# szemenyeim/DynEnv

Measured on AMD Instinct MI355X. Metric: agent-steps/s, higher is better.
Workload: dtype f64

## Files before the change

dynenv_amd/csrc/driving_kernels.hip:

```cpp
#include "driving_dev.h"

__constant__ DrvConst C;

#include "driving_host.h"

struct DrvMailbox {
  double p1x[DRV_NS][2], p1y[DRV_NS][2], p2x[DRV_NS][2], p2y[DRV_NS][2], nx[DRV_NS], ny[DRV_NS];
  int hash[DRV_NS][2], count[DRV_NS], flag[DRV_NS];
};
struct DrvObsStage {
  float carRow[DRV_MAXA][8];
  float goal[DRV_MAXA][2];
  float shared[DRV_MAXO * 4 + DRV_MAXP * 2 + DRV_LANE_ROWS * 5];
};
#ifdef DRV_PROFILE
#define DRV_PROF(...) __VA_ARGS__
#else
#define DRV_PROF(...)
#endif
#define DRV_CLIST 128
struct __align__(16) DrvLds {
  double px[DRV_NB], py[DRV_NB], vx[DRV_NB], vy[DRV_NB], ang[DRV_NB], w[DRV_NB], vbx[DRV_NB], vby[DRV_NB], wb[DRV_NB];
  double minv[DRV_NB], iinv[DRV_NB];
  double rc[DRV_MAXA], rs[DRV_MAXA], rotAng[DRV_MAXA];
  double dirx[DRV_MAXA], diry[DRV_MAXA], prevx[DRV_MAXA], prevy[DRV_MAXA], goalx[DRV_MAXA], goaly[DRV_MAXA];
  double cosRel0[DRV_MAXA];
  double dprev[DRV_MAXA];
  double cmass[DRV_MAXA], cpower[DRV_MAXA], chx[DRV_MAXA], chy[DRV_MAXA];
  double aabb[DRV_MAXA][4];
  V2 cv[DRV_MAXA][4];
  int flags[DRV_NB], moving[DRV_NB];
  double ox[DRV_MAXO], oy[DRV_MAXO];
  int s_pair[DRV_NS], s_meta[DRV_NS], s_hash0[DRV_NS], s_hash1[DRV_NS];
  double s_jn0[DRV_NS], s_jt0[DRV_NS], s_jn1[DRV_NS], s_jt1[DRV_NS];
  double rewAcc[DRV_MAXA], posAcc[DRV_MAXA];
  int lastCand[64];
  int stepErr;
  unsigned char act[16];
  int still[DRV_NB];
  unsigned short clist[DRV_CLIST];
  int clistN;
  int sLvMeta;
  unsigned long long sActive;
  unsigned char sLevel[DRV_NS];
  union {
    DrvMailbox mb;
    DrvObsStage ob;
  } u;
};

static_assert(sizeof(DrvLds) <= 10240, "16 one-wave workgroups per CU - one residency round of 4096 environments on 256 CUs - need <= 160 KB / 16 of LDS each");
__shared__ DrvLds g_L;


#define DRV_COS_PI_2 6.123233995736766e-17
template <int R>
struct RoadK;
template <>
struct RoadK<0> {
  static constexpr double p0x = 875.0, p0y = 0.0, dirx = 0.0, diry = 1.0, lat = 2.0 * 35.0 + 5.0, length = 1000.0;
  static constexpr double dirAngle = 1.5707963267948966, cosDir0 = DRV_COS_PI_2, nx = -1.0, ny = DRV_COS_PI_2;
};
template <>
struct RoadK<1> {
  static constexpr double p0x = 0.0, p0y = 500.0, dirx = 1.0, diry = 0.0, lat = 1.0 * 35.0 + 5.0, length = 1750.0;
  static constexpr double dirAngle = 0.0, cosDir0 = 1.0, nx = DRV_COS_PI_2, ny = 1.0;
};

struct CarK {
  static constexpr double carMass0 = 1200.0, carMass1 = 1800.0, carMass2 = 3500.0, carMass3 = 5000.0;
  static constexpr double carHx0 = 10.0, carHx1 = 15.0, carHx2 = 20.0, carHx3 = 25.0;
  static constexpr double carHy0 = 5.0, carHy1 = 6.0, carHy2 = 7.0, carHy3 = 8.0;
  static constexpr double carPower0 = 3.0, carPower1 = 4.0, carPower2 = 3.0, carPower3 = 4.0;
  static constexpr double carInertia0 = 50000.0, carInertia1 = 156600.0, carInertia2 = 0x1.ff8e555555555p+18, carInertia3 = 0x1.185ad55555555p+20;
  static constexpr double pedMass = 90.0, pedInertia = 90.0 * (0.5 * (0.0 * 0.0 + DRV_PED_R * DRV_PED_R) + 0.0);
};

template <int R>
DE_DEV int road_pos(V2 point, double cosRel) {
  V2 pt = vsub(point, v2(RoadK<R>::p0x, RoadK<R>::p0y));
  double dist = vcross(v2(RoadK<R>::dirx, RoadK<R>::diry), pt);
// ... 746 lines not shown
      if (active && myLevel == lv && a_state != ARB_FIRST) {
        BodyV a, b;
        body_load(L, bodyA, a);
        body_load(L, bodyB, b);
        arb_warm_start(a, b, n, r1, r2, jn, jt, a_count);
        body_store_vel(L, bodyA, a);
        body_store_vel(L, bodyB, b);
      }
      __syncthreads();
    }
    BodyV a, b;
    bool biasOnly = true;
    if (active) {
      body_load(L, bodyA, a); body_load(L, bodyB, b);
      biasOnly = arb_is_bias_only(a, b, jn, jt, bounce, a_count);
    }
    const int nSteps = maxLevel + 1 + period * 9;
    int due = myLevel, passes = 0;
DRV_PROF(profMode = wave_ballot(!biasOnly) == 0ull ? 3 : 4;)
    if (wave_ballot(!biasOnly) == 0ull) {
      const int ra = body_rd(bodyA), rb = body_rd(bodyB), wa = body_wr(bodyA), wb_ = body_wr(bodyB);
      for (int t = 0; t < nSteps; ++t) {
        if (active && t == due && passes < 10) {
          a.vb = v2(L.vbx[ra], L.vby[ra]); a.wb = L.wb[ra];
          b.vb = v2(L.vbx[rb], L.vby[rb]); b.wb = L.wb[rb];
          arb_apply_bias_only(a, b, n, r1, r2, nMass, bias, jBias, a_count);
          L.vbx[wa] = a.vb.x; L.vby[wa] = a.vb.y; L.wb[wa] = a.wb;
          L.vbx[wb_] = b.vb.x; L.vby[wb_] = b.vb.y; L.wb[wb_] = b.wb;
          due += period; ++passes;
        }
        __syncthreads();
      }
    } else [[unlikely]] {
DRV_PROF(if (lane == 0 && blockIdx.x < 4096) { unsigned long long* d = g_dbgp + blockIdx.x * 8; const unsigned long long P3 = __builtin_amdgcn_s_memtime(); d[2] += P1 - P0; d[3] += (P2 - P1) + ((P3 - P2) << 32); })
      const int bits3 = (restIn ? B3_REST_IN : 0) | (bias[0] == 0.0 ? B3_BIAS0_ZERO : 0) | (bias[1] == 0.0 ? B3_BIAS1_ZERO : 0);
      DrvSolveRet r;
      r[0] = nMass[0]; r[1] = nMass[1]; r[2] = bias[0]; r[3] = bias[1]; r[4] = bounce[0]; r[5] = bounce[1];
      r[6] = jn[0]; r[7] = jn[1]; r[8] = jt[0]; r[9] = jt[1];
      r[10] = drv_pack2(pk, a_pair);
      r[11] = drv_pack2(SOLVE_NEEDS_SPLIT | (bits3 << SR_BITS3_SH) | (myLevel << SR_LEVEL_SH), bodyA | (bodyB << 8) | (maxLevel_ << SR_LVWORD_SH));
      return r;
    }
  }
DRV_PROF(const unsigned long long P3 = __builtin_amdgcn_s_memtime();)
  const int bits = drv_slot_verdicts(lane, pk, a_pair, restIn, bias[0] == 0.0, bias[1] == 0.0, jn[0], jn[1], jt[0], jt[1], jBias[0], jBias[1], false);
DRV_PROF(if (lane == 0 && blockIdx.x < 4096) { unsigned long long* d = g_dbgp + blockIdx.x * 8; const unsigned long long P4 = __builtin_amdgcn_s_memtime(); d[2] += (P1 - P0) + ((P4 - P3) << 32); d[3] += (P2 - P1) + ((P3 - P2) << 32); })
  DrvSolveRet r;
  r[11] = drv_pack2(bits DRV_PROF(| (prof_any(profMode) << SOLVE_PROF_SH)), 0);
  return r;
}
DE_OOL int drv_prestep_solve(int lane, int nCarPed, int pk, int a_pair, int bodyA, int bodyB, int anyActive_, double jn0, double jn1, double jt0,
                             double jt1) {
  return __double2loint(drv_prestep_solve_body<false>(lane, nCarPed, pk, a_pair, bodyA, bodyB, 0, 1 << 8 , anyActive_, jn0, jn1, jt0, jt1)[11]);
}
DE_OOL DrvSolveRet drv_prestep_solve_multi(int lane, int nCarPed, int pk, int a_pair, int bodyA, int bodyB, int myLevel, int maxLevel_, double jn0,
                                           double jn1, double jt0, double jt1) {
  return drv_prestep_solve_body<true>(lane, nCarPed, pk, a_pair, bodyA, bodyB, myLevel, maxLevel_, 1, jn0, jn1, jt0, jt1);
}
DE_OOL int drv_split_verdicts(int lane, int pk, int a_pair, int bits3, double jn0, double jn1, double jBias0, double jBias1, double jt0, double jt1) {
  return drv_slot_verdicts(lane, pk, a_pair, (bits3 & B3_REST_IN) != 0, (bits3 & B3_BIAS0_ZERO) != 0, (bits3 & B3_BIAS1_ZERO) != 0, jn0, jn1, jt0, jt1, jBias0, jBias1, true);
}
enum { CRET_OVERFLOW = 1, CRET_INERT_SH = 1, CRET_INERT = 1 << CRET_INERT_SH, CRET_STEADY_SH = 2, CRET_STEADY = 1 << CRET_STEADY_SH,
       CRET_LIGHT_REPLAY_SH = 3, CRET_LIGHT_REPLAY = 1 << CRET_LIGHT_REPLAY_SH, CRET_SPLIT_SH = 4, CRET_SPLIT = 1 << CRET_SPLIT_SH };
static_assert(SOLVE_ALL_INERT == CRET_INERT && SOLVE_ALL_STEADY == CRET_STEADY && (SOLVE_TOOK_SPLIT << 1) == CRET_SPLIT,
              "drv_contact_path passes the two verdicts on in place and the split bit one place up");
struct ContactRet {
  uint64_t occ;
  int err;
};

DE_DEV ContactRet drv_contact_path(int lane, int cand, int dirty, int light, int A, int nCarPed, uint64_t occ) {
  const bool isCar = lane < A, isPed = lane >= DRV_SLOT_PED && lane < DRV_SLOT_PED + (nCarPed >> 8);
  DrvLds& L = g_L;
  int err = 0;
  asm volatile("" : "+v"(lane));
DRV_PROF(const unsigned long long T0 = __builtin_amdgcn_s_memtime();)
  DrvMailbox& M = L.u.mb;
  if (lane < DRV_NS) M.flag[lane] = 0;
  __syncthreads();
// ... 67 lines not shown
    if (mode == 0) { lightBad = lightBad || touch; continue; }
    const uint64_t tmask = wave_ballot(touch);
    if (tmask == 0ull) continue;
    const bool needNew = touch && slot < 0;
    const uint64_t newMask = wave_ballot(needNew);
    if (newMask) {
      const uint64_t slotBits = (1ull << DRV_NS) - 1ull;
      int rank = __popcll(newMask & ((1ull << lane) - 1ull));
      uint64_t fm = (~occ) & slotBits;
      if (needNew) {
        for (int r = 0; r < rank; ++r) fm &= fm - 1;
        if (fm) { slot = __builtin_ctzll(fm); L.s_pair[slot] = pr; }
        else err |= CRET_OVERFLOW;
      }
      int cnt = __popcll(newMask);
      uint64_t fm2 = (~occ) & slotBits;
      for (int r = 0; r < cnt && fm2; ++r) { occ |= (fm2 & (~fm2 + 1)); fm2 &= fm2 - 1; }
      spair = lane < DRV_NS ? L.s_pair[lane] : -1;
    }
    if (touch && slot >= 0) {
      M.flag[slot] = needNew ? 3 : 1;
      M.count[slot] = ct.count;
      M.nx[slot] = ct.n.x; M.ny[slot] = ct.n.y;
      M.p1x[slot][0] = ct.p1[0].x; M.p1y[slot][0] = ct.p1[0].y; M.p2x[slot][0] = ct.p2[0].x; M.p2y[slot][0] = ct.p2[0].y;
      M.hash[slot][0] = ct.hash[0];
      if (ct.count > 1) {
        M.p1x[slot][1] = ct.p1[1].x; M.p1y[slot][1] = ct.p1[1].y; M.p2x[slot][1] = ct.p2[1].x; M.p2y[slot][1] = ct.p2[1].y;
        M.hash[slot][1] = ct.hash[1];
      }
    }
    __syncthreads();
  }
  __syncthreads();
DRV_PROF(if (lane == 0 && blockIdx.x < 4096) { unsigned long long* d = g_dbgl + blockIdx.x * 8; d[6] += (N1 - T0) + (nMath << 32); d[7] += __builtin_amdgcn_s_memtime() - N1 - nMath; })
  if (mode == 0 && wave_ballot(lightBad) == 0ull) { lightOk = true; break; }
  }
  if (lightOk) {
    ContactRet ret;
    ret.occ = occ; ret.err = err | CRET_LIGHT_REPLAY;
    return ret;
  }

DRV_PROF(const unsigned long long T1 = __builtin_amdgcn_s_memtime();)
  const bool slotOcc = lane < DRV_NS && ((occ >> lane) & 1ull);
  bool touched = false;
  int bodyA = 0, bodyB = 0;
  int a_pair = 0xFFFF, a_state = ARB_FIRST, a_count = 0, a_age = 0;
  bool hashSame = false;
  bool prevSteady = false, prevInert = false;
  double jn[2] = {0.0, 0.0}, jt[2] = {0.0, 0.0};
  V2 n = v2(0.0, 0.0), r1[2], r2[2];
  r1[0] = r1[1] = r2[0] = r2[1] = v2(0.0, 0.0);
  const int sl = lane < DRV_NS ? lane : 0;
  int flag = M.flag[sl], cnt = M.count[sl], h0 = M.hash[sl][0], mh1 = M.hash[sl][1];
  int s_pair = L.s_pair[sl], meta = L.s_meta[sl], oh0 = L.s_hash0[sl], oh1 = L.s_hash1[sl];
  double o_jn0 = L.s_jn0[sl], o_jt0 = L.s_jt0[sl], o_jn1 = L.s_jn1[sl], o_jt1 = L.s_jt1[sl];
  asm volatile("" : "+v"(flag), "+v"(cnt), "+v"(h0), "+v"(mh1), "+v"(s_pair), "+v"(meta), "+v"(oh0), "+v"(oh1), "+v"(o_jn0), "+v"(o_jt0), "+v"(o_jn1), "+v"(o_jt1));
  if (slotOcc) {
    touched = flag != 0;
    a_pair = s_pair;
    a_state = SLOT_STATE(meta); a_count = SLOT_COUNT(meta); a_age = SLOT_AGE(meta);
    prevSteady = SLOT_BIT(meta, META_STEADY_SH); prevInert = SLOT_BIT(meta, META_INERT_SH);
    if (flag & 2) { a_state = ARB_FIRST; a_count = 0; a_age = 0; prevSteady = false; prevInert = false; }
    if (touched) {
      const int i = a_pair >> 8, j = a_pair & 0xFF;
      if (j >= DRV_SLOT_PED && j < DRV_SLOT_OBST) { bodyA = j; bodyB = i; } else { bodyA = i; bodyB = j; }
      const V2 pa = bodyA < DRV_SLOT_OBST ? v2(L.px[bodyA], L.py[bodyA]) : static_pos(L, bodyA);
// ... 104 lines not shown
  else if (nActive > 1 && lvHit) {
    myLevel = c_level;
    maxLevel = (int)(signed char)(uniform_i(c_meta) & 0xFF);
    period = uniform_i(c_meta) >> 8;
  } else if (nActive > 1) {
    if (!haveRank && nTouched > 1)
      for (uint64_t mm = touchedMask; mm; mm &= mm - 1) {
        int b = __builtin_ctzll(mm);
        int pk = bcast_i(a_pair, b);
        rank += (pk < a_pair) ? 1 : 0;
      }
    int bl = 0;
    const int bodyAB = bodyA | (bodyB << 8);
    for (int k = 0; k < nTouched; ++k) {
      uint64_t who = wave_ballot(active && rank == k);
      if (who == 0ull) continue;
      int b = __builtin_ctzll(who);
      const int ab = bcast_i(bodyAB, b), ba = ab & 0xFF, bb2 = ab >> 8;
      const int pa = ba < DRV_SLOT_OBST ? bcast_i(bl, ba) : 0, pb = bb2 < DRV_SLOT_OBST ? bcast_i(bl, bb2) : 0;
      const int la = pa & 0xFF, lb = pb & 0xFF;
      int lv = la > lb ? la : lb;
      const int fa = (pa >> 8) - 1, fb = (pb >> 8) - 1;
      const int lo = fa < 0 ? fb : (fb < 0 ? fa : (fa < fb ? fa : fb));
      if (lo >= 0 && lv - lo + 1 > period) period = lv - lo + 1;
      if (lane == b) myLevel = lv;
      if (lane == ba || lane == bb2) bl = (lv + 1) | (((bl >> 8) ? (bl >> 8) : lv + 1) << 8);
      maxLevel = lv > maxLevel ? lv : maxLevel;
    }
    if (lane < DRV_NS) L.sLevel[lane] = (unsigned char)myLevel;
    if (lane == 0) L.sLvMeta = (maxLevel & 0xFF) | (period << 8);
  }

DRV_PROF(const unsigned long long T2 = __builtin_amdgcn_s_memtime();)
DRV_PROF(if (lane == 0 && blockIdx.x < 4096) { unsigned long long* d = g_dbgs + blockIdx.x * 8; d[0] += U1 - T1; d[1] += U2 - U1; d[2] += U3 - U2; d[3] += U4 - U3; d[4] += T2 - U4; })
  const int pkArg = pk_pack(a_state, a_count, a_age, touched, freeMe, hashSame, prevInert, skipped, slotOcc, active);
  int solveBits;
  if (activeMask == 0ull || maxLevel == 0) {
    solveBits = drv_prestep_solve(lane, nCarPed, pkArg, a_pair, bodyA, bodyB, activeMask != 0ull ? 1 : 0, jn[0], jn[1], jt[0], jt[1]);
  } else {
    const DrvSolveRet sv = drv_prestep_solve_multi(lane, nCarPed, pkArg, a_pair, bodyA, bodyB, myLevel, (maxLevel & 0xFF) | (period << 8), jn[0], jn[1], jt[0], jt[1]);
    solveBits = __double2loint(sv[11]);
    if (uniform_i(solveBits) & SOLVE_NEEDS_SPLIT) [[unlikely]] {
      const int w1 = __double2hiint(sv[11]);
DRV_PROF(const unsigned long long S0 = __builtin_amdgcn_s_memtime();)
      const DrvSplitRet sr = drv_solve_general_split(fresh_lane(), (solveBits >> SR_LEVEL_SH) & 0xFF, w1 & 0xFFFF, w1 >> SR_LVWORD_SH, sv[0], sv[1], sv[2], sv[3], sv[4], sv[5],
                                                     sv[6], sv[7], sv[8], sv[9], __double2loint(sv[10]), __double2hiint(sv[10]), (solveBits >> SR_BITS3_SH) & 7);
DRV_PROF(const unsigned long long S1 = __builtin_amdgcn_s_memtime();)
      solveBits = drv_split_verdicts(fresh_lane(), sr.pk, sr.pair, sr.bits, sr.jn0, sr.jn1, sr.jb0, sr.jb1, sr.jt0, sr.jt1) DRV_PROF(| (4 << SOLVE_PROF_SH));
DRV_PROF(if (fresh_lane() == 0 && blockIdx.x < 4096) { unsigned long long* d = g_dbgp + blockIdx.x * 8; d[3] += (S1 - S0) << 32; d[2] += (__builtin_amdgcn_s_memtime() - S1) << 32; })
    }
  }
  occ &= ~freeMask;
DRV_PROF(const unsigned long long T3 = T2, T4 = T2, T5 = __builtin_amdgcn_s_memtime(); const int profModeW = (uniform_i(solveBits) >> SOLVE_PROF_SH) & 7;)
DRV_PROF(if (lane == 0 && blockIdx.x < 4096) {
  unsigned long long* d = g_dbgp + blockIdx.x * 8;
  d[0] += T1 - T0; d[1] += T2 - T1; d[2] += T3 - T2; d[3] += T4 - T3; d[4] += T5 - T4;
  d[5] += 1ull + (light ? (1ull << 16) : 0ull);
  d[6] += (unsigned long long)(maxLevel + 1) + ((unsigned long long)(maxLevel + 1) << (12 * profModeW));
  d[7] += (unsigned long long)nTouched + ((unsigned long long)profCand << 16);
})
  {
    ContactRet ret;
    ret.occ = occ; ret.err = err | (uniform_i(solveBits) & (SOLVE_ALL_INERT | SOLVE_ALL_STEADY)) | ((uniform_i(solveBits) & SOLVE_TOOK_SPLIT) << 1);
    return ret;
  }
}

DE_OOL int drv_partial_obs_fused(PvIn in, uint64_t seed, int A, int* envi, int env_id_offset, int e, int nPedObst, int elapsed,
                                 uint32_t episode, int noiseTypeAgents, double magn, float* __restrict__ obs, int budgetCycles);
#ifndef DRV_DEFER_MIN_CONTACT
#define DRV_DEFER_MIN_CONTACT 5
#endif
#ifndef DRV_PV_DEADLINE_PCT
#define DRV_PV_DEADLINE_PCT 110
#endif
#ifndef DRV_FUSED_AGENTS
#define DRV_FUSED_AGENTS 10
#endif
enum { LR_MOVING = 1, LR_REMOVED = 2, LR_CAND_CHANGED = 4 };
enum { LS_VB_VALID = 1, LS_AABB_VALID = 2 };
struct DrvLightRet {
  int cand, dirty, bits;
};
DE_OOL DrvLightRet drv_light_substep(int it_, int lane, int A_, int nPed_, int nObst_, int elapsed_,
                                                      uint32_t seedLo, uint32_t seedHi, uint32_t genv_, uint32_t episode_, int stateBits) {
  DrvLds& L = g_L;
DRV_PROF(const unsigned long long Q0 = __builtin_amdgcn_s_memtime();)
  const int lastCand = L.lastCand[lane];
  const int it = uniform_i(it_), A = uniform_i(A_), nPed = uniform_i(nPed_), nObst = uniform_i(nObst_), elapsed = uniform_i(elapsed_);
  const uint32_t genv = (uint32_t)uniform_i((int)genv_), episode = (uint32_t)uniform_i((int)episode_);
  const uint64_t seed = ((uint64_t)(uint32_t)uniform_i((int)seedHi) << 32) | (uint64_t)(uint32_t)uniform_i((int)seedLo);
  const bool isCar = lane < A;
  const bool isPed = lane >= DRV_SLOT_PED && lane < DRV_SLOT_PED + nPed;
  const bool isBody = isCar || isPed;
  const bool vbValid = (uniform_i(stateBits) & LS_VB_VALID) != 0;
  bool aabbValid = (uniform_i(stateBits) & LS_AABB_VALID) != 0;
    bool turned = false;
    const int bi = lane & (DRV_NB - 1), ci = lane < DRV_MAXA ? lane : DRV_MAXA - 1;
    int f = L.flags[bi];
    double px = L.px[bi], py = L.py[bi], vx = L.vx[bi], vy = L.vy[bi], ang = L.ang[bi];
    const double w = L.w[bi];
    const double vbx = vbValid ? L.vbx[bi] : 0.0, vby = vbValid ? L.vby[bi] : 0.0, wb = vbValid ? L.wb[bi] : 0.0;
    double rcv = L.rc[ci], rsv = L.rs[ci], rotAngv = L.rotAng[ci], cosRel0v = L.cosRel0[ci];
    const double goalx = L.goalx[ci], goaly = L.goaly[ci], dprev = L.dprev[ci], chx = L.chx[ci], chy = L.chy[ci];
    double rew = L.rewAcc[ci], posrew = L.posAcc[ci];
    int moving = L.moving[bi];
    if (!isBody) { f = 0; px = 0.0; py = 0.0; vx = 0.0; vy = 0.0; }
    if (isCar) {
      if (it == 0) {
        const int actPk = (int)L.act[lane];
        const int acc = (actPk & 3) - 1, steer = ((actPk >> 2) - 1) * 2;
        if (!CARF_FIN(f)) {
          double dirx = L.dirx[lane], diry = L.diry[lane];
          double power = (double)acc;
          double moveDir = vx * dirx + vy * diry;
          bool skip = false;
          if (acc < 0) power = (double)acc * 0.75;
          if (acc == 0) power = (moveDir == 0.0) ? 0.0 : (moveDir > 0.0 ? -2.0 : 2.0);
          else if (acc < 0 && moveDir > 0.0) skip = true;
          else if (acc > 0 && moveDir < 0.0) skip = true;
          if (!skip) {
            const double cs = rcv, sn = rsv;
            const double cpower = L.cpower[lane];
            vx = vx + cpower * power * cs;
            vy = vy + cpower * power * sn;
            if (acc == 0 && (vx * dirx + vy * diry) * moveDir < 0.0) { vx = 0.0; vy = 0.0; }
          }
          if (steer != 0) {
            const double rot = (double)steer * (DM_PI / 180.0);
            ang = ang + rot;
            const DevSC rsc = dev_sincos_inl(rot);
            const double sn = rsc.s, cs = rsc.c;
            const double dx = dirx * cs - diry * sn, dy = dirx * sn + diry * cs;
            L.dirx[lane] = dx; L.diry[lane] = dy;
            const double nvx = vx * cs - vy * sn, nvy = vx * sn + vy * cs;
            vx = nvx; vy = nvy;
            L.ang[lane] = ang;
            const CarRot cr = car_refresh_rot<true>(L, lane, ang);
            rcv = cr.c; rsv = cr.s; rotAngv = ang; cosRel0v = cr.cosRel0;
            turned = true;
// ... 4 lines not shown
DRV_PROF(const unsigned long long Q1 = __builtin_amdgcn_s_memtime();)
    const V2 pos = v2(px, py);
    int lp = LP_OffRoad;
    if (isBody) {
      int rp = road_pos<0>(pos, isCar ? cosRel0v : RoadK<0>::cosDir0);
      if (rp < lp) lp = rp;
      rp = road_pos<1>(pos, isCar ? rcv : RoadK<1>::cosDir0);
      if (rp < lp) lp = rp;
    }
DRV_PROF(const unsigned long long Q2 = __builtin_amdgcn_s_memtime();)
    if (isCar) {
      const double dnow = vlen(vsub(pos, v2(goalx, goaly)));
      const double diff = dprev - dnow;
      if (!CARF_FIN(f)) { const double d50 = diff / 50.0; rew += d50; posrew += dm_max(0.0, d50); }
      L.prevx[lane] = px; L.prevy[lane] = py; L.dprev[lane] = dnow;
      if (lp >= LP_OverRoad) {
        if (!CARF_FIN(f)) {
          if (lp == LP_OverRoad && dnow < 100.0) {
            lp = LP_AtGoal;
            f |= CARF_FIN_BIT | CARF_FRIC_BIT;
            rew += (double)(DRV_MAX_TIME - elapsed) / 100.0;
            posrew += (double)(DRV_MAX_TIME - elapsed) / 100.0;
          } else {
            f |= CARF_CRASH_BITS;
            rew -= vlen(v2(vx, vy)) / 5.0;
          }
        }
      } else if (lp == LP_InOpposingLane) {
        if (!CARF_FIN(f)) rew -= vlen(v2(vx, vy)) / 10000.0;
      }
      f = CARF_SET_LP(f, lp);
      if (px >= DRV_W + 50.0 || px <= -50.0 || py >= DRV_H + 50.0 || py <= -50.0) { vx = 0.0; vy = 0.0; }
      L.flags[lane] = f;
      L.vx[lane] = vx; L.vy[lane] = vy;
      L.rewAcc[lane] = rew; L.posAcc[lane] = posrew;
DRV_PROF(asm volatile("" ::: "memory");)
    } else if (isPed) {
      if (!PEDF_DEAD(f)) {
        int crossing = PEDF_CROSSING(f), beginc = PEDF_BEGIN(f), side = PEDF_SIDE(f);
        const bool isOffRoad = lp >= LP_OverRoad;
        const bool isOut = drv_is_out(pos);
        if (moving > 0) {
          moving = (moving - DRV_TIME_DIFF > 0) ? moving - DRV_TIME_DIFF : 0;
          if (crossing) {
            if (!beginc && isOffRoad) { moving = 0; crossing = 0; vx = 0.0; vy = 0.0; }
            else if (beginc && !isOffRoad) { beginc = 0; }
          }
          if (isOut) { moving = 0; vx = 0.0; vy = 0.0; }
        } else {
          if (!crossing) {
            dm_u32x4 u = dm_env_rng(seed, genv, episode, DM_RNG_PED_MOVE, (uint32_t)(lane - DRV_SLOT_PED), (uint32_t)elapsed);
            const bool r1 = PEDF_ROAD(f) != 0;
            const V2 rdir = r1 ? v2(RoadK<1>::dirx, RoadK<1>::diry) : v2(RoadK<0>::dirx, RoadK<0>::diry);
            const V2 rnrm = r1 ? v2(RoadK<1>::nx, RoadK<1>::ny) : v2(RoadK<0>::nx, RoadK<0>::ny);
            V2 dir = rdir;
            moving = dm_randint(u.v[0], 5000, 30000);
            int speed = dm_randint(u.v[1], -2, 2);
            if (!isOffRoad) {
              crossing = 1; beginc = 0;
              if (speed == 0) speed = 2;
            } else if (isOut) {
              dir = drv_is_out(vadd(pos, rdir)) ? vneg(rdir) : rdir;
            } else if (dm_unit(u.v[2]) < 0.05) {
              crossing = 1; beginc = 1;
              dir = side ? rnrm : vneg(rnrm);
              side = side ? 0 : 1;
              speed = dm_randint(u.v[3], 1, 2);
            }
            const V2 nv = vmul(vmul(dir, (double)PEDF_SPEED(f)), (double)speed);
            vx = nv.x; vy = nv.y;
          } else if (isOffRoad) {
            crossing = 0; beginc = 0;
          }
        }
        L.moving[lane] = moving;
        L.flags[lane] = PEDF_PACK(PEDF_ROAD(f), side, 0, crossing, beginc, PEDF_SPEED(f));
        L.vx[lane] = vx; L.vy[lane] = vy;
      }
    }

DRV_PROF(const unsigned long long Q3 = __builtin_amdgcn_s_memtime();)
    double bl = 0.0, bb = 0.0, br = -1.0, bt = -1.0;
    bool live = false;
    int sj = 3;
    if (isBody) {
      const double npx = px + (vx + vbx) * DE_DT, npy = py + (vy + vby) * DE_DT, nang = ang + (w + wb) * DE_DT;
      const bool still = !turned && vx == 0.0 && vy == 0.0 && w == 0.0 && vbx == 0.0 && vby == 0.0 && wb == 0.0;
      L.px[lane] = npx; L.py[lane] = npy; L.ang[lane] = nang;
      const bool frozen = !turned && vx == 0.0 && vy == 0.0 && w == 0.0 && npx == px && npy == py && nang == ang;
      sj = (still ? 1 : 0) | (frozen ? 2 : 0);
      L.still[lane] = sj;
      live = true;
      if (isCar) {
        if (nang != rotAngv) { const CarRot cr = car_refresh_rot<true>(L, lane, nang); rcv = cr.c; rsv = cr.s; }
        if (!aabbValid || !frozen) {
          BoxW bw;
          box_world(bw, v2(npx, npy), rcv, rsv, chx, chy);
          double l = INFINITY, r = -INFINITY, b = INFINITY, t = -INFINITY;
#pragma unroll
          for (int k = 0; k < 4; ++k) {
            l = fmin_cp(l, bw.v[k].x); r = fmax_cp(r, bw.v[k].x); b = fmin_cp(b, bw.v[k].y); t = fmax_cp(t, bw.v[k].y);
          }
          bl = l - 0.0; bb = b - 0.0; br = r + 0.0; bt = t + 0.0;
#pragma unroll
          for (int k = 0; k < 4; ++k) L.cv[lane][k] = bw.v[k];
          L.aabb[lane][0] = bl; L.aabb[lane][1] = bb; L.aabb[lane][2] = br; L.aabb[lane][3] = bt;
        } else {
          bl = L.aabb[lane][0]; bb = L.aabb[lane][1]; br = L.aabb[lane][2]; bt = L.aabb[lane][3];
        }
      } else {
// ... 1 lines not shown
      }
    } else if (lane >= DRV_SLOT_OBST && lane < DRV_SLOT_BLD + 4) {
      live = lane >= DRV_SLOT_BLD || (lane - DRV_SLOT_OBST) < nObst;
      const V2 c = static_pos(L, lane);
      const double ex = lane >= DRV_SLOT_BLD ? DRV_BLD_HX : DRV_OBST_H, ey = lane >= DRV_SLOT_BLD ? DRV_BLD_HY : DRV_OBST_H;
      bl = -ex + c.x; br = ex + c.x; bb = -ey + c.y; bt = ey + c.y;
    }
    aabbValid = true;
    __syncthreads();
DRV_PROF(const unsigned long long Q4 = __builtin_amdgcn_s_memtime();)

    int cand = 0;
    bool candMoving = false, removed = false;
    int dirty = 0;
    {
      const int carStill = (int)(wave_ballot(isCar && (sj & 1)) & 0x3FFull);
      const int carFrozen = (int)(wave_ballot(isCar && (sj & 2)) & 0x3FFull);
#pragma unroll
      for (int i = 0; i < DRV_MAXA; ++i) {
        const double al = L.aabb[i][0], ab = L.aabb[i][1], ar = L.aabb[i][2], at = L.aabb[i][3];
        const bool hit = (al <= br) & (bl <= ar) & (ab <= bt) & (bb <= at);
        cand |= hit ? (1 << i) : 0;
      }
      {
        const int lim = lane < A ? lane : A;
        cand &= live ? ((1 << lim) - 1) : 0;
      }
      if (cand) candMoving = !(sj & 1) || (cand & ~carStill) != 0;
      const int clean = (lastCand >= 0 && (sj & 2)) ? (cand & lastCand & carFrozen) : 0;
      dirty = cand & ~clean;
      removed = lastCand < 0 || (lastCand & ~cand) != 0;
    }
  L.lastCand[lane] = cand;
DRV_PROF(if (lane == 0 && blockIdx.x < 4096) {
  unsigned long long* d = g_dbgl + blockIdx.x * 8;
  const unsigned long long Q5 = __builtin_amdgcn_s_memtime();
  if (it == 0) { for (int k = 0; k < 8; ++k) d[k] = 0ull; }
  d[0] += Q1 - Q0; d[1] += Q2 - Q1; d[2] += Q3 - Q2; d[3] += Q4 - Q3; d[4] += Q5 - Q4; d[5] += Q5 - Q0;
})
  DrvLightRet ret;
  ret.cand = cand; ret.dirty = dirty; ret.bits = (candMoving ? LR_MOVING : 0) | (removed ? LR_REMOVED : 0) | (cand != lastCand ? LR_CAND_CHANGED : 0);
  return ret;
}
DE_DEV unsigned drv_hw_simd_key() {
  const unsigned hw = (unsigned)__builtin_amdgcn_s_getreg(63492) , xcc = (unsigned)__builtin_amdgcn_s_getreg(63508) ;
  return ((xcc & 0xFu) << 16) | (hw & 0xFF30u);
}
DE_DEV int drv_launch_tick(const DrvState& S) { return S.tick_src ? uniform_i(__atomic_load_n(&S.iso[DRV_ISOW_TICK], __ATOMIC_RELAXED)) : S.tick; }
DE_DEV int drv_launch_pv(const DrvState& S) { return S.tick_src ? uniform_i(__atomic_load_n(&S.iso[DRV_ISOW_PV_PAR], __ATOMIC_RELAXED)) : S.pv_par; }
DE_DEV int drv_iso_assign(const DrvState& S, int lane, int tick) {
  const int b = blockIdx.x, E = S.E;
  if (!S.iso_on) return b;
  const int buf = tick % 3;
  if (b == 0 && lane == 0) { const int nn = (tick + 2) % 3; S.iso[DRV_ISOW_LEN + nn] = 0; S.iso[DRV_ISOW_SLOWEST + nn] = 0; }
  if (S.iso_on == 3) return b;
  int K = uniform_i(S.iso[DRV_ISOW_LEN + buf]);
  const int cap = S.iso_on == 1 ? DRV_ISO_MAX : DRV_ISO_LIST;
  K = K < cap ? K : cap;
  const int G = S.iso_on == 1 ? 4 * DRV_ISO_GROUPS : E;
  if (S.iso_on == 1) {
    if (b < G) { if (lane == 0) S.iso_hw[(size_t)(tick & 1) * (4 * DRV_ISO_GROUPS) + b] = drv_hw_simd_key(); }
    else if (b == G + 3 * DRV_ISO_MAX) {
      const unsigned* hw = S.iso_hw + (size_t)((tick + 1) & 1) * (4 * DRV_ISO_GROUPS);
      bool bad = false;
      for (int g = DRV_ISO_G0 + lane; g < DRV_ISO_G0 + DRV_ISO_GSPAN; g += 64) {
        const unsigned k0 = hw[g], k1 = hw[g + DRV_ISO_GROUPS], k2 = hw[g + 2 * DRV_ISO_GROUPS], k3 = hw[g + 3 * DRV_ISO_GROUPS];
        bad |= k0 == 0xFFFFFFFFu || k0 != k1 || k0 != k2 || k0 != k3;
      }
      const bool ok = wave_ballot(bad) == 0ull;
      if (lane == 0) {
        int cd = S.iso[DRV_ISOW_COOL];
        if (!ok) cd = DRV_ISO_COOLDOWN; else if (cd > 0) cd -= 1;
        S.iso[DRV_ISOW_COOL] = cd;
        S.iso[DRV_ISOW_VALID + (tick + 1) % 3] = (ok && cd == 0) ? 1 : 0;
// ... 47 lines not shown
#endif
#ifndef DRV_ISO_PCT
#define DRV_ISO_PCT 75
#endif
DE_DEV void drv_iso_report(const DrvState& S, int e, int lane, unsigned long long t0, int tick) {
  if (!S.iso_on || lane != 0) return;
  const int cycles = (int)(__builtin_amdgcn_s_memtime() - t0);
  const int buf = tick % 3, nxt = (tick + 1) % 3;
  const int slowest = S.iso[DRV_ISOW_SLOWEST + buf];
  if (cycles > DRV_ISO_MIN && cycles > (slowest / 100) * DRV_ISO_PCT) atomicMax(&S.iso[DRV_ISOW_SLOWEST + nxt], cycles);
  if (S.iso_on == 3) return;
  if (slowest > DRV_ISO_MIN && cycles > (slowest / 100) * DRV_ISO_PCT) {
    const int k = atomicAdd(&S.iso[DRV_ISOW_LEN + nxt], 1);
    if (k < DRV_ISO_LIST) S.iso[DRV_ISO_HDR + nxt * DRV_ISO_LIST + k] = e;
  }
  __atomic_store_n(&S.iso_done[e], tick, __ATOMIC_RELAXED);
}

template <bool PARTIAL>
DE_DEV void drv_step_body(const DrvState& S, const uint8_t* __restrict__ mask, const int* __restrict__ actions, float* __restrict__ obs,
                          double* __restrict__ rewards, uint8_t* __restrict__ dones, float* __restrict__ pobs, int pvNoise, double pvMagn) {
  const unsigned long long isoT0 = __builtin_amdgcn_s_memtime();
DRV_PROF(const unsigned long long KS = isoT0;)
  DrvLds& L = g_L;
  int lane = threadIdx.x;
  const int tick = drv_launch_tick(S);
  if (!S.tick_src && blockIdx.x == 0 && lane == 0) { S.iso[DRV_ISOW_TICK] = S.tick; S.iso[DRV_ISOW_PV_PAR] = S.pv_par; }
  const int e = drv_iso_assign(S, lane, tick);
  if (e < 0) return;
  if (mask && uniform_i(mask[e]) == 0) {
    if ((S.iso_on == 1 || S.iso_on == 2) && lane == 0) __atomic_store_n(&S.iso_done[e], tick, __ATOMIC_RELAXED);
    return;
  }
DRV_PROF(if (lane < 8 && e < 4096) { g_dbgp[e * 8 + lane] = 0ull; g_dbgs[e * 8 + lane] = 0ull; })
  const int A = S.A;
  int* envi = S.envi + (size_t)e * EI_COUNT;
  int elapsed = uniform_i(envi[EI_ELAPSED]);
  int allFinished = uniform_i(envi[EI_ALLFIN]);
  const int nPed = uniform_i(envi[EI_NPED]);
  const int nObst = uniform_i(envi[EI_NOBST]);
  const uint32_t episode = (uint32_t)uniform_i(envi[EI_EPISODE]);
  uint64_t occ = (uint64_t)(uint32_t)uniform_i(envi[EI_OCC]);
  if (occ != 0ull) __builtin_amdgcn_s_setprio(3);
  else if (PARTIAL) __builtin_amdgcn_s_setprio(1);
  const uint32_t genv = (uint32_t)(S.env_id_offset + e);

  const bool isCar = lane < A;
  const bool isPed = lane >= DRV_SLOT_PED && lane < DRV_SLOT_PED + nPed;
  const bool isBody = isCar || isPed;
  const int g_act0 = actions[((size_t)e * A + (isCar ? lane : 0)) * 2 + 0], g_act1 = actions[((size_t)e * A + (isCar ? lane : 0)) * 2 + 1];
  const int g_lastCand = S.lastcand[(size_t)e * 64 + lane];
  load_env(S, L, e, lane, A, nPed, nObst, occ);

  {
    int act0 = isCar ? g_act0 : 1, act1 = isCar ? g_act1 : 1;
    const bool bad = (unsigned)act0 > 2u || (unsigned)act1 > 2u;
    if (bad) { act0 = 1; act1 = 1; }
    if (lane < 16) L.act[lane] = (unsigned char)(act0 | (act1 << 2));
    const bool anyBad = wave_ballot(bad) != 0ull;
    if (lane == 0) L.stepErr = anyBad ? DYNENV_ERRBIT_ACTION : 0;
  }
  int finishedAt = -1;
  if (lane < DRV_MAXA) { L.rewAcc[lane] = 0.0; L.posAcc[lane] = 0.0; }
  bool aabbValid = false;
  L.lastCand[lane] = g_lastCand;
  if (lane == 0) { L.clistN = -1; L.sActive = ~0ull; L.sLvMeta = 0; }
  bool inertAll = (uniform_i(envi[EI_SHORTCUT]) & SC_INERT) != 0;
  bool steadyAll = (uniform_i(envi[EI_SHORTCUT]) & SC_STEADY) != 0;
  bool vbValid = (uniform_i(envi[EI_SHORTCUT]) & SC_VB_VALID) != 0;
  unsigned cntA = 0u, cntB = 0u;
#define DRV_CNT(ei) (1u << (4 * ((ei) - EI_N_FAST)))
#define DRV_CNT_GET(ei) ((int)((cntA >> (4 * ((ei) - EI_N_FAST))) & 15u))
  static_assert(EI_N_STEADY - EI_N_FAST == 7 && EI_N_SLOTS - EI_N_FAST == 3 && DRV_NS * 10 < 256, "seven counters of four bits in cntA, the slot sum in eight bits of cntB");
  __syncthreads();

DRV_PROF(const unsigned long long K0 = __builtin_amdgcn_s_memtime(); unsigned long long tPh1 = 0, tBroad = 0, tFast = 0, tCont = 0, tBook = 0;)
  bool lightOff = false;
  for (int it = 0; it < 10; ++it) {
    lane = fresh_lane();
DRV_PROF(const unsigned long long A0 = __builtin_amdgcn_s_memtime();)
    const DrvLightRet lr = drv_light_substep(it, lane, A, nPed, nObst, elapsed, (uint32_t)S.seed, (uint32_t)(S.seed >> 32), genv, episode,
                                             (vbValid ? LS_VB_VALID : 0) | (aabbValid ? LS_AABB_VALID : 0));
    const int cand = lr.cand, dirty = lr.dirty;
    const bool candMoving = (lr.bits & LR_MOVING) != 0, removed = (lr.bits & LR_REMOVED) != 0;
    aabbValid = true;
DRV_PROF(const unsigned long long A1 = A0;)
    const uint64_t anyCand = wave_ballot(cand != 0);
    const bool candChanged = wave_ballot((lr.bits & LR_CAND_CHANGED) != 0) != 0ull, anyMoving = wave_ballot(candMoving) != 0ull;
    if (candChanged && lane == 0) L.clistN = -1;
    const bool quiescent = inertAll && !candChanged && !anyMoving;
    const bool steadyOk = !quiescent && steadyAll && wave_ballot(removed) == 0ull;
    const bool anyDirty = wave_ballot(dirty != 0) != 0ull;
    bool replay = steadyOk && !anyDirty;
    const bool light = steadyOk && anyDirty && !lightOff;
    if (!(anyCand == 0ull && occ == 0ull) && !quiescent && !replay) cntA += candChanged ? DRV_CNT(EI_N_WHY_CAND) : anyMoving ? DRV_CNT(EI_N_WHY_MOVING) : DRV_CNT(EI_N_WHY_INERT);

DRV_PROF(const unsigned long long A2 = __builtin_amdgcn_s_memtime(); bool tookContact = false;)
    cntA += (anyCand == 0ull && occ == 0ull) ? DRV_CNT(EI_N_FAST) : quiescent ? DRV_CNT(EI_N_QUIET) : replay ? DRV_CNT(EI_N_STEADY) : DRV_CNT(EI_N_CONTACT);
    cntB += (unsigned)__popcll(occ);
    if ((anyCand == 0ull && occ == 0ull) || quiescent) {
      velocity_update_ool(A | (nPed << 8));
      if (anyCand == 0ull && occ == 0ull) steadyAll = false;
      vbValid = false;
    } else if (!replay) {
DRV_PROF(tookContact = true;)
      __builtin_amdgcn_s_setprio(3);
      ContactRet cr = drv_contact_path(lane, cand, dirty, light ? 1 : 0, A, A | (nPed << 8), occ);
      lane = fresh_lane();
      if (wave_ballot((cr.err & CRET_OVERFLOW) != 0) != 0ull && lane == 0) L.stepErr |= DYNENV_ERRBIT_OVERFLOW;
      if (light && !(uniform_i(cr.err >> CRET_LIGHT_REPLAY_SH) & 1)) lightOff = true;
      if (uniform_i(cr.err >> CRET_LIGHT_REPLAY_SH) & 1) {
        replay = true; cntB = (unsigned)uniform_i((int)(cntB + (1u << 8)));
      } else {
        cntB = (unsigned)uniform_i((int)(cntB + ((unsigned)(uniform_i(cr.err >> CRET_SPLIT_SH) & 1) << 12)));
        occ = uniform_u64(cr.occ);
        inertAll = (uniform_i(cr.err >> CRET_INERT_SH) & 1) != 0;
        steadyAll = (uniform_i(cr.err >> CRET_STEADY_SH) & 1) != 0;
        vbValid = true;
      }
    }
    if (replay) {
      velocity_update_ool(A | (nPed << 8));
      vbValid = true;
    }
    __syncthreads();
    if (!PARTIAL) lane = fresh_lane();

DRV_PROF(const unsigned long long A3 = __builtin_amdgcn_s_memtime(); tPh1 += A1 - A0; tBroad += A2 - A1; if (tookContact) tCont += A3 - A2; else tFast += A3 - A2;)
    elapsed += 1;
    bool notDone = false;
    if (isCar) { int f = L.flags[lane]; notDone = !(CARF_FIN(f) && !CARF_CRASHED(f)); }
    const bool allFin = wave_ballot(notDone) == 0ull;
    if (!allFinished && allFin) {
      allFinished = 1;
      finishedAt = elapsed;
    }
  }
  lane = fresh_lane();
  const double teamReward = finishedAt >= 0 ? 0.0 + (double)(DRV_MAX_TIME - finishedAt) / 100.0 : 0.0;

DRV_PROF(const unsigned long long K1 = __builtin_amdgcn_s_memtime();)
  double* er = S.epr + (size_t)e * 16 + (isCar ? lane : 0);
  double* ep = S.epr + (size_t)S.E * 16 + (size_t)e * 16 + (isCar ? lane : 0);
  const double g_er = *er, g_ep = *ep;
  const int cl = lane < 10 ? lane : 0;
  const int g_cnt = envi[EI_N_FAST + cl];
  const int g_err = envi[EI_ERR];
  double rew = 0.0, posrew = 0.0;
  if (isCar) {
    rew = L.rewAcc[lane] + teamReward;
    posrew = L.posAcc[lane] + dm_max(0.0, teamReward);
    rewards[(size_t)e * A + lane] = rew;
  }
  if (lane == 0) {
    dones[e] = (uint8_t)(elapsed >= DRV_MAX_TIME);
    envi[EI_ELAPSED] = elapsed; envi[EI_ALLFIN] = allFinished; envi[EI_OCC] = (int)(uint32_t)occ;
    envi[EI_SHORTCUT] = (inertAll ? SC_INERT : 0) | (steadyAll ? SC_STEADY : 0) | (vbValid ? SC_VB_VALID : 0);
  }
  const int errBits = uniform_i(L.stepErr);
  S.lastcand[(size_t)e * 64 + lane] = L.lastCand[lane];
  store_env(S, L, e, lane, A, nPed, occ);
  if (obs) write_full_obs_ool(lane, A, nPed, nObst, S.obs_dim, obs + (size_t)e * A * S.obs_dim);
  if (isCar) { *er = g_er + rew; *ep = g_ep + posrew; }
  {
    static_assert(EI_N_QUIET == EI_N_FAST + 1 && EI_N_CONTACT == EI_N_FAST + 2 && EI_N_SLOTS == EI_N_FAST + 3 && EI_N_WHY_CAND == EI_N_FAST + 4 &&
                  EI_N_WHY_MOVING == EI_N_FAST + 5 && EI_N_WHY_INERT == EI_N_FAST + 6 && EI_N_STEADY == EI_N_FAST + 7 && EI_N_LIGHT == EI_N_FAST + 8 && EI_N_SPLIT == EI_N_FAST + 9,
// ... 215 lines not shown
```

Before: 272.9 million.

## Fuse velocity update and path decisions into light substep, drop per-step barrier

The velocity/friction update for the fast, quiescent and replay paths now runs inside the light substep, and that function computes the wave-uniform path decision bits. This removes a separate out-of-line velocity_update call, the vx/vy round trip through LDS, and the per-iteration __syncthreads. The all-finished check is deferred to the next substep through a ballot on previous flags, plus one final check after the loop. The profiling index now comes from an LDS env id instead of blockIdx. The risk is subtle ordering changes: w is written before the broadphase reads it, and correctness now depends on a compiler memory barrier rather than an explicit sync.

```diff
diff --git a/dynenv_amd/csrc/driving_kernels.hip b/dynenv_amd/csrc/driving_kernels.hip
--- a/dynenv_amd/csrc/driving_kernels.hip
+++ b/dynenv_amd/csrc/driving_kernels.hip
@@ -47,6 +47,7 @@
     DrvMailbox mb;
     DrvObsStage ob;
   } u;
+DRV_PROF(int profEnv;)
 };
 
 static_assert(sizeof(DrvLds) <= 10240, "16 one-wave workgroups per CU - one residency round of 4096 environments on 256 CUs - need <= 160 KB / 16 of LDS each");
@@ -859,7 +860,7 @@
         __syncthreads();
       }
     } else [[unlikely]] {
-DRV_PROF(if (lane == 0 && blockIdx.x < 4096) { unsigned long long* d = g_dbgp + blockIdx.x * 8; const unsigned long long P3 = __builtin_amdgcn_s_memtime(); d[2] += P1 - P0; d[3] += (P2 - P1) + ((P3 - P2) << 32); })
+DRV_PROF(if (lane == 0 && g_L.profEnv < 4096) { unsigned long long* d = g_dbgp + g_L.profEnv * 8; const unsigned long long P3 = __builtin_amdgcn_s_memtime(); d[2] += P1 - P0; d[3] += (P2 - P1) + ((P3 - P2) << 32); })
       const int bits3 = (restIn ? B3_REST_IN : 0) | (bias[0] == 0.0 ? B3_BIAS0_ZERO : 0) | (bias[1] == 0.0 ? B3_BIAS1_ZERO : 0);
       DrvSolveRet r;
       r[0] = nMass[0]; r[1] = nMass[1]; r[2] = bias[0]; r[3] = bias[1]; r[4] = bounce[0]; r[5] = bounce[1];
@@ -871,7 +872,7 @@
   }
 DRV_PROF(const unsigned long long P3 = __builtin_amdgcn_s_memtime();)
   const int bits = drv_slot_verdicts(lane, pk, a_pair, restIn, bias[0] == 0.0, bias[1] == 0.0, jn[0], jn[1], jt[0], jt[1], jBias[0], jBias[1], false);
-DRV_PROF(if (lane == 0 && blockIdx.x < 4096) { unsigned long long* d = g_dbgp + blockIdx.x * 8; const unsigned long long P4 = __builtin_amdgcn_s_memtime(); d[2] += (P1 - P0) + ((P4 - P3) << 32); d[3] += (P2 - P1) + ((P3 - P2) << 32); })
+DRV_PROF(if (lane == 0 && g_L.profEnv < 4096) { unsigned long long* d = g_dbgp + g_L.profEnv * 8; const unsigned long long P4 = __builtin_amdgcn_s_memtime(); d[2] += (P1 - P0) + ((P4 - P3) << 32); d[3] += (P2 - P1) + ((P3 - P2) << 32); })
   DrvSolveRet r;
   r[11] = drv_pack2(bits DRV_PROF(| (prof_any(profMode) << SOLVE_PROF_SH)), 0);
   return r;
@@ -1005,7 +1006,7 @@
     __syncthreads();
   }
   __syncthreads();
-DRV_PROF(if (lane == 0 && blockIdx.x < 4096) { unsigned long long* d = g_dbgl + blockIdx.x * 8; d[6] += (N1 - T0) + (nMath << 32); d[7] += __builtin_amdgcn_s_memtime() - N1 - nMath; })
+DRV_PROF(if (lane == 0 && g_L.profEnv < 4096) { unsigned long long* d = g_dbgl + g_L.profEnv * 8; d[6] += (N1 - T0) + (nMath << 32); d[7] += __builtin_amdgcn_s_memtime() - N1 - nMath; })
   if (mode == 0 && wave_ballot(lightBad) == 0ull) { lightOk = true; break; }
   }
   if (lightOk) {
@@ -1176,7 +1177,7 @@
   }
 
 DRV_PROF(const unsigned long long T2 = __builtin_amdgcn_s_memtime();)
-DRV_PROF(if (lane == 0 && blockIdx.x < 4096) { unsigned long long* d = g_dbgs + blockIdx.x * 8; d[0] += U1 - T1; d[1] += U2 - U1; d[2] += U3 - U2; d[3] += U4 - U3; d[4] += T2 - U4; })
+DRV_PROF(if (lane == 0 && g_L.profEnv < 4096) { unsigned long long* d = g_dbgs + g_L.profEnv * 8; d[0] += U1 - T1; d[1] += U2 - U1; d[2] += U3 - U2; d[3] += U4 - U3; d[4] += T2 - U4; })
   const int pkArg = pk_pack(a_state, a_count, a_age, touched, freeMe, hashSame, prevInert, skipped, slotOcc, active);
   int solveBits;
   if (activeMask == 0ull || maxLevel == 0) {
@@ -1191,13 +1192,13 @@
                                                      sv[6], sv[7], sv[8], sv[9], __double2loint(sv[10]), __double2hiint(sv[10]), (solveBits >> SR_BITS3_SH) & 7);
 DRV_PROF(const unsigned long long S1 = __builtin_amdgcn_s_memtime();)
       solveBits = drv_split_verdicts(fresh_lane(), sr.pk, sr.pair, sr.bits, sr.jn0, sr.jn1, sr.jb0, sr.jb1, sr.jt0, sr.jt1) DRV_PROF(| (4 << SOLVE_PROF_SH));
-DRV_PROF(if (fresh_lane() == 0 && blockIdx.x < 4096) { unsigned long long* d = g_dbgp + blockIdx.x * 8; d[3] += (S1 - S0) << 32; d[2] += (__builtin_amdgcn_s_memtime() - S1) << 32; })
+DRV_PROF(if (fresh_lane() == 0 && g_L.profEnv < 4096) { unsigned long long* d = g_dbgp + g_L.profEnv * 8; d[3] += (S1 - S0) << 32; d[2] += (__builtin_amdgcn_s_memtime() - S1) << 32; })
     }
   }
   occ &= ~freeMask;
 DRV_PROF(const unsigned long long T3 = T2, T4 = T2, T5 = __builtin_amdgcn_s_memtime(); const int profModeW = (uniform_i(solveBits) >> SOLVE_PROF_SH) & 7;)
-DRV_PROF(if (lane == 0 && blockIdx.x < 4096) {
-  unsigned long long* d = g_dbgp + blockIdx.x * 8;
+DRV_PROF(if (lane == 0 && g_L.profEnv < 4096) {
+  unsigned long long* d = g_dbgp + g_L.profEnv * 8;
   d[0] += T1 - T0; d[1] += T2 - T1; d[2] += T3 - T2; d[3] += T4 - T3; d[4] += T5 - T4;
   d[5] += 1ull + (light ? (1ull << 16) : 0ull);
   d[6] += (unsigned long long)(maxLevel + 1) + ((unsigned long long)(maxLevel + 1) << (12 * profModeW));
@@ -1221,8 +1222,8 @@
 #ifndef DRV_FUSED_AGENTS
 #define DRV_FUSED_AGENTS 10
 #endif
-enum { LR_MOVING = 1, LR_REMOVED = 2, LR_CAND_CHANGED = 4 };
-enum { LS_VB_VALID = 1, LS_AABB_VALID = 2 };
+enum { LR_PREV_ALLFIN = 1, LR_FAST = 2, LR_QUIET = 4, LR_REPLAY = 8, LR_CAND_CHANGED = 16, LR_ANY_MOVING = 32, LR_STEADY_OK = 64, LR_ANY_DIRTY = 128 };
+enum { LS_VB_VALID = 1, LS_AABB_VALID = 2, LS_OCC = 4, LS_INERT = 8, LS_STEADY = 16 };
 struct DrvLightRet {
   int cand, dirty, bits;
 };
@@ -1243,13 +1244,16 @@
     const int bi = lane & (DRV_NB - 1), ci = lane < DRV_MAXA ? lane : DRV_MAXA - 1;
     int f = L.flags[bi];
     double px = L.px[bi], py = L.py[bi], vx = L.vx[bi], vy = L.vy[bi], ang = L.ang[bi];
-    const double w = L.w[bi];
-    const double vbx = vbValid ? L.vbx[bi] : 0.0, vby = vbValid ? L.vby[bi] : 0.0, wb = vbValid ? L.wb[bi] : 0.0;
+    double w = L.w[bi];
+    const double l_vbx = L.vbx[bi], l_vby = L.vby[bi], l_wb = L.wb[bi];
+    const double cmass = L.cmass[ci];
     double rcv = L.rc[ci], rsv = L.rs[ci], rotAngv = L.rotAng[ci], cosRel0v = L.cosRel0[ci];
     const double goalx = L.goalx[ci], goaly = L.goaly[ci], dprev = L.dprev[ci], chx = L.chx[ci], chy = L.chy[ci];
     double rew = L.rewAcc[ci], posrew = L.posAcc[ci];
     int moving = L.moving[bi];
+    const double vbx = vbValid ? l_vbx : 0.0, vby = vbValid ? l_vby : 0.0, wb = vbValid ? l_wb : 0.0;
     if (!isBody) { f = 0; px = 0.0; py = 0.0; vx = 0.0; vy = 0.0; }
+    const bool prevAllFin = wave_ballot(isCar && !(CARF_FIN(f) && !CARF_CRASHED(f))) == 0ull;
     if (isCar) {
       if (it == 0) {
         const int actPk = (int)L.act[lane];
@@ -1320,7 +1324,6 @@
       f = CARF_SET_LP(f, lp);
       if (px >= DRV_W + 50.0 || px <= -50.0 || py >= DRV_H + 50.0 || py <= -50.0) { vx = 0.0; vy = 0.0; }
       L.flags[lane] = f;
-      L.vx[lane] = vx; L.vy[lane] = vy;
       L.rewAcc[lane] = rew; L.posAcc[lane] = posrew;
 DRV_PROF(asm volatile("" ::: "memory");)
     } else if (isPed) {
@@ -1363,7 +1366,6 @@
         }
         L.moving[lane] = moving;
         L.flags[lane] = PEDF_PACK(PEDF_ROAD(f), side, 0, crossing, beginc, PEDF_SPEED(f));
-        L.vx[lane] = vx; L.vy[lane] = vy;
       }
     }
 
@@ -1431,14 +1433,36 @@
       removed = lastCand < 0 || (lastCand & ~cand) != 0;
     }
   L.lastCand[lane] = cand;
-DRV_PROF(if (lane == 0 && blockIdx.x < 4096) {
-  unsigned long long* d = g_dbgl + blockIdx.x * 8;
+  const bool occAny = (uniform_i(stateBits) & LS_OCC) != 0, inertAll = (uniform_i(stateBits) & LS_INERT) != 0, steadyAll = (uniform_i(stateBits) & LS_STEADY) != 0;
+  const bool candChanged = wave_ballot(cand != lastCand) != 0ull, anyMoving = wave_ballot(candMoving) != 0ull;
+  if (candChanged && lane == 0) L.clistN = -1;
+  const bool fast = wave_ballot(cand != 0) == 0ull && !occAny;
+  const bool quiescent = inertAll && !candChanged && !anyMoving;
+  const bool steadyOk = !quiescent && steadyAll && wave_ballot(removed) == 0ull;
+  const bool anyDirty = wave_ballot(dirty != 0) != 0ull;
+  const bool replay = !fast && steadyOk && !anyDirty;
+  if (isBody) {
+    if (fast || quiescent || replay) {
+      double m, fr, rfr;
+      bool dflt = false;
+      if (isCar) { m = cmass; fr = CARF_FRIC(f) ? 5e-4 : 5e-5; rfr = CARF_FRIC(f) ? 2e-5 : 1e-5; }
+      else { m = CarK::pedMass; fr = 5e-2; rfr = 2e-4; dflt = !PEDF_DEAD(f); }
+      if (dflt) { vx = vx * 1.0 + (0.0 + 0.0) * DE_DT; vy = vy * 1.0 + (0.0 + 0.0) * DE_DT; w = w * 1.0 + 0.0; }
+      else apply_friction(vx, vy, w, m, fr, rfr, 0.0);
+      L.w[lane] = w;
+    }
+    L.vx[lane] = vx; L.vy[lane] = vy;
+  }
+DRV_PROF(if (lane == 0 && g_L.profEnv < 4096) {
+  unsigned long long* d = g_dbgl + g_L.profEnv * 8;
   const unsigned long long Q5 = __builtin_amdgcn_s_memtime();
   if (it == 0) { for (int k = 0; k < 8; ++k) d[k] = 0ull; }
   d[0] += Q1 - Q0; d[1] += Q2 - Q1; d[2] += Q3 - Q2; d[3] += Q4 - Q3; d[4] += Q5 - Q4; d[5] += Q5 - Q0;
 })
   DrvLightRet ret;
-  ret.cand = cand; ret.dirty = dirty; ret.bits = (candMoving ? LR_MOVING : 0) | (removed ? LR_REMOVED : 0) | (cand != lastCand ? LR_CAND_CHANGED : 0);
+  ret.cand = cand; ret.dirty = dirty;
+  ret.bits = (prevAllFin ? LR_PREV_ALLFIN : 0) | (fast ? LR_FAST : 0) | (quiescent && !fast ? LR_QUIET : 0) | (replay && !quiescent ? LR_REPLAY : 0) |
+             (candChanged ? LR_CAND_CHANGED : 0) | (anyMoving ? LR_ANY_MOVING : 0) | (steadyOk ? LR_STEADY_OK : 0) | (anyDirty ? LR_ANY_DIRTY : 0);
   return ret;
 }
 DE_DEV unsigned drv_hw_simd_key() {
@@ -1552,7 +1576,7 @@
     if ((S.iso_on == 1 || S.iso_on == 2) && lane == 0) __atomic_store_n(&S.iso_done[e], tick, __ATOMIC_RELAXED);
     return;
   }
-DRV_PROF(if (lane < 8 && e < 4096) { g_dbgp[e * 8 + lane] = 0ull; g_dbgs[e * 8 + lane] = 0ull; })
+DRV_PROF(if (lane == 0) L.profEnv = e; if (lane < 8 && e < 4096) { g_dbgp[e * 8 + lane] = 0ull; g_dbgs[e * 8 + lane] = 0ull; })
   const int A = S.A;
   int* envi = S.envi + (size_t)e * EI_COUNT;
   int elapsed = uniform_i(envi[EI_ELAPSED]);
@@ -1600,29 +1624,29 @@
     lane = fresh_lane();
 DRV_PROF(const unsigned long long A0 = __builtin_amdgcn_s_memtime();)
     const DrvLightRet lr = drv_light_substep(it, lane, A, nPed, nObst, elapsed, (uint32_t)S.seed, (uint32_t)(S.seed >> 32), genv, episode,
-                                             (vbValid ? LS_VB_VALID : 0) | (aabbValid ? LS_AABB_VALID : 0));
+                                             (vbValid ? LS_VB_VALID : 0) | (aabbValid ? LS_AABB_VALID : 0) | (occ != 0ull ? LS_OCC : 0) |
+                                             (inertAll ? LS_INERT : 0) | (steadyAll ? LS_STEADY : 0));
     const int cand = lr.cand, dirty = lr.dirty;
-    const bool candMoving = (lr.bits & LR_MOVING) != 0, removed = (lr.bits & LR_REMOVED) != 0;
+    const int lb = uniform_i(lr.bits);
     aabbValid = true;
+    if (it > 0 && !allFinished && (lb & LR_PREV_ALLFIN)) {
+      allFinished = 1;
+      finishedAt = elapsed;
+    }
 DRV_PROF(const unsigned long long A1 = A0;)
-    const uint64_t anyCand = wave_ballot(cand != 0);
-    const bool candChanged = wave_ballot((lr.bits & LR_CAND_CHANGED) != 0) != 0ull, anyMoving = wave_ballot(candMoving) != 0ull;
-    if (candChanged && lane == 0) L.clistN = -1;
-    const bool quiescent = inertAll && !candChanged && !anyMoving;
-    const bool steadyOk = !quiescent && steadyAll && wave_ballot(removed) == 0ull;
-    const bool anyDirty = wave_ballot(dirty != 0) != 0ull;
-    bool replay = steadyOk && !anyDirty;
-    const bool light = steadyOk && anyDirty && !lightOff;
-    if (!(anyCand == 0ull && occ == 0ull) && !quiescent && !replay) cntA += candChanged ? DRV_CNT(EI_N_WHY_CAND) : anyMoving ? DRV_CNT(EI_N_WHY_MOVING) : DRV_CNT(EI_N_WHY_INERT);
+    const bool fast = (lb & LR_FAST) != 0, quiescent = (lb & LR_QUIET) != 0, replay = (lb & LR_REPLAY) != 0;
+    const bool light = (lb & LR_STEADY_OK) && (lb & LR_ANY_DIRTY) && !lightOff;
+    if (!fast && !quiescent && !replay) cntA += (lb & LR_CAND_CHANGED) ? DRV_CNT(EI_N_WHY_CAND) : (lb & LR_ANY_MOVING) ? DRV_CNT(EI_N_WHY_MOVING) : DRV_CNT(EI_N_WHY_INERT);
 
 DRV_PROF(const unsigned long long A2 = __builtin_amdgcn_s_memtime(); bool tookContact = false;)
-    cntA += (anyCand == 0ull && occ == 0ull) ? DRV_CNT(EI_N_FAST) : quiescent ? DRV_CNT(EI_N_QUIET) : replay ? DRV_CNT(EI_N_STEADY) : DRV_CNT(EI_N_CONTACT);
+    cntA += fast ? DRV_CNT(EI_N_FAST) : quiescent ? DRV_CNT(EI_N_QUIET) : replay ? DRV_CNT(EI_N_STEADY) : DRV_CNT(EI_N_CONTACT);
     cntB += (unsigned)__popcll(occ);
-    if ((anyCand == 0ull && occ == 0ull) || quiescent) {
-      velocity_update_ool(A | (nPed << 8));
-      if (anyCand == 0ull && occ == 0ull) steadyAll = false;
+    if (fast || quiescent) {
+      if (fast) steadyAll = false;
       vbValid = false;
-    } else if (!replay) {
+    } else if (replay) {
+      vbValid = true;
+    } else {
 DRV_PROF(tookContact = true;)
       __builtin_amdgcn_s_setprio(3);
       ContactRet cr = drv_contact_path(lane, cand, dirty, light ? 1 : 0, A, A | (nPed << 8), occ);
@@ -1630,28 +1654,25 @@
       if (wave_ballot((cr.err & CRET_OVERFLOW) != 0) != 0ull && lane == 0) L.stepErr |= DYNENV_ERRBIT_OVERFLOW;
       if (light && !(uniform_i(cr.err >> CRET_LIGHT_REPLAY_SH) & 1)) lightOff = true;
       if (uniform_i(cr.err >> CRET_LIGHT_REPLAY_SH) & 1) {
-        replay = true; cntB = (unsigned)uniform_i((int)(cntB + (1u << 8)));
+        cntB = (unsigned)uniform_i((int)(cntB + (1u << 8)));
+        velocity_update_ool(A | (nPed << 8));
       } else {
         cntB = (unsigned)uniform_i((int)(cntB + ((unsigned)(uniform_i(cr.err >> CRET_SPLIT_SH) & 1) << 12)));
         occ = uniform_u64(cr.occ);
         inertAll = (uniform_i(cr.err >> CRET_INERT_SH) & 1) != 0;
         steadyAll = (uniform_i(cr.err >> CRET_STEADY_SH) & 1) != 0;
-        vbValid = true;
-      }
-    }
-    if (replay) {
-      velocity_update_ool(A | (nPed << 8));
+      }
       vbValid = true;
     }
-    __syncthreads();
-    if (!PARTIAL) lane = fresh_lane();
-
+    asm volatile("" ::: "memory");
 DRV_PROF(const unsigned long long A3 = __builtin_amdgcn_s_memtime(); tPh1 += A1 - A0; tBroad += A2 - A1; if (tookContact) tCont += A3 - A2; else tFast += A3 - A2;)
     elapsed += 1;
+  }
+  lane = fresh_lane();
+  {
     bool notDone = false;
-    if (isCar) { int f = L.flags[lane]; notDone = !(CARF_FIN(f) && !CARF_CRASHED(f)); }
-    const bool allFin = wave_ballot(notDone) == 0ull;
-    if (!allFinished && allFin) {
+    if (lane < A) { const int f = L.flags[lane]; notDone = !(CARF_FIN(f) && !CARF_CRASHED(f)); }
+    if (!allFinished && wave_ballot(notDone) == 0ull) {
       allFinished = 1;
       finishedAt = elapsed;
     }
```

Result: faster. 276.1 million, median of 6 (+1.2%).
